# jayleicn/ClipBERT

Measured on NVIDIA H100. Metric: clips/sec fwd+bwd MSRVTT ret (ResNet50+BERT-base), higher is better.
Workload: dtype bf16

## Files before the change

clipbert_b200/csrc/common.cuh:

```cuda
#pragma once
#include <cuda.h>
#include <cuda_bf16.h>
#include <cuda_runtime.h>
#include <stdint.h>

#include "drop_cfg.h"

namespace cb {

#ifndef CB_SPIN_LIMIT
#define CB_SPIN_LIMIT (1u << 24)
#endif

__device__ __forceinline__ uint32_t smem_u32(const void* p) {
  return static_cast<uint32_t>(__cvta_generic_to_shared(p));
}

__device__ __forceinline__ void pdl_wait() { asm volatile("griddepcontrol.wait;" ::: "memory"); }
__device__ __forceinline__ void pdl_trigger() { asm volatile("griddepcontrol.launch_dependents;" ::: "memory"); }

__device__ __forceinline__ void mbar_init(uint64_t* bar, uint32_t count) {
  asm volatile("mbarrier.init.shared::cta.b64 [%0], %1;" ::"r"(smem_u32(bar)), "r"(count));
}
__device__ __forceinline__ void fence_mbar_init() {
// ... 28 lines not shown
}
__device__ __forceinline__ void mbar_wait(uint64_t* bar, uint32_t parity) {
  uint32_t spins = 0;
  while (!mbar_try_wait(bar, parity)) {
    if (++spins > CB_SPIN_LIMIT) __trap();
  }
}
__device__ __forceinline__ void mbar_wait_unguarded(uint64_t* bar, uint32_t parity) {
  while (!mbar_try_wait(bar, parity)) {
  }
}

__device__ __forceinline__ void tma_prefetch_desc(const CUtensorMap* map) {
  asm volatile("prefetch.tensormap [%0];" ::"l"(map) : "memory");
}
__device__ __forceinline__ void tma_load_2d(void* smem_dst, const CUtensorMap* map, uint64_t* bar,
                                            int c0, int c1) {
  asm volatile(
      "cp.async.bulk.tensor.2d.shared::cluster.global.mbarrier::complete_tx::bytes "
      "[%0], [%1, {%3, %4}], [%2];" ::"r"(smem_u32(smem_dst)),
      "l"(map), "r"(smem_u32(bar)), "r"(c0), "r"(c1)
      : "memory");
}

__device__ __forceinline__ void bulk_load_1d(uint32_t smem_dst, const void* gsrc, uint32_t bytes, uint64_t* bar) {
  asm volatile("cp.async.bulk.shared::cluster.global.mbarrier::complete_tx::bytes [%0], [%1], %2, [%3];" ::"r"(smem_dst), "l"(gsrc),
               "r"(bytes), "r"(smem_u32(bar))
               : "memory");
}

__device__ __forceinline__ void tma_load_2d_s32(uint32_t smem_dst, const CUtensorMap* map, uint64_t* bar, int c0, int c1) {
  asm volatile(
      "cp.async.bulk.tensor.2d.shared::cluster.global.mbarrier::complete_tx::bytes "
      "[%0], [%1, {%3, %4}], [%2];" ::"r"(smem_dst),
      "l"(map), "r"(smem_u32(bar)), "r"(c0), "r"(c1)
      : "memory");
}

__device__ __forceinline__ void tma_load_3d(void* smem_dst, const CUtensorMap* map, uint64_t* bar, int c0, int c1, int c2) {
  asm volatile(
      "cp.async.bulk.tensor.3d.shared::cluster.global.mbarrier::complete_tx::bytes "
      "[%0], [%1, {%3, %4, %5}], [%2];" ::"r"(smem_u32(smem_dst)),
      "l"(map), "r"(smem_u32(bar)), "r"(c0), "r"(c1), "r"(c2)
      : "memory");
}

__device__ __forceinline__ void tma_store_2d(const CUtensorMap* map, const void* smem_src, int c0, int c1) {
  asm volatile("cp.async.bulk.tensor.2d.global.shared::cta.bulk_group [%0, {%2, %3}], [%1];" ::"l"(map),
               "r"(smem_u32(smem_src)), "r"(c0), "r"(c1)
               : "memory");
}
__device__ __forceinline__ void tma_store_2d_s32(const CUtensorMap* map, uint32_t smem_src, int c0, int c1) {
  asm volatile("cp.async.bulk.tensor.2d.global.shared::cta.bulk_group [%0, {%2, %3}], [%1];" ::"l"(map), "r"(smem_src), "r"(c0), "r"(c1)
               : "memory");
}
__device__ __forceinline__ uint4 lds128(uint32_t saddr) {
  uint4 v;
  asm volatile("ld.shared.v4.u32 {%0, %1, %2, %3}, [%4];" : "=r"(v.x), "=r"(v.y), "=r"(v.z), "=r"(v.w) : "r"(saddr));
  return v;
}
__device__ __forceinline__ void sts128(uint32_t saddr, uint4 v) {
  asm volatile("st.shared.v4.u32 [%0], {%1, %2, %3, %4};" ::"r"(saddr), "r"(v.x), "r"(v.y), "r"(v.z), "r"(v.w) : "memory");
}
__device__ __forceinline__ void tma_store_commit() { asm volatile("cp.async.bulk.commit_group;" ::: "memory"); }
template <int N>
__device__ __forceinline__ void tma_store_wait_read() {
  asm volatile("cp.async.bulk.wait_group.read %0;" ::"n"(N) : "memory");
}
template <int N>
__device__ __forceinline__ void tma_store_wait_all() {
  asm volatile("cp.async.bulk.wait_group %0;" ::"n"(N) : "memory");
}
__device__ __forceinline__ void named_bar_sync(uint32_t id, uint32_t nthreads) {
  asm volatile("bar.sync %0, %1;" ::"r"(id), "r"(nthreads) : "memory");
}
__device__ __forceinline__ void named_bar_arrive(uint32_t id, uint32_t nthreads) {
  asm volatile("bar.arrive %0, %1;" ::"r"(id), "r"(nthreads) : "memory");
}
template <uint32_t NREG>
__device__ __forceinline__ void setmaxnreg_dec() {
  asm volatile("setmaxnreg.dec.sync.aligned.u32 %0;" ::"n"(NREG));
}
template <uint32_t NREG>
__device__ __forceinline__ void setmaxnreg_inc() {
  asm volatile("setmaxnreg.inc.sync.aligned.u32 %0;" ::"n"(NREG));
}

__device__ __forceinline__ void wgmma_fence() { asm volatile("wgmma.fence.sync.aligned;" ::: "memory"); }
__device__ __forceinline__ void wgmma_commit() { asm volatile("wgmma.commit_group.sync.aligned;" ::: "memory"); }
template <int N>
__device__ __forceinline__ void wgmma_wait() {
  asm volatile("wgmma.wait_group.sync.aligned %0;" ::"n"(N) : "memory");
}
template <int R>
__device__ __forceinline__ void wgmma_fence_acc(float (&d)[R]) {
#pragma unroll
  for (int i = 0; i < R; ++i) asm volatile("" : "+f"(d[i])::"memory");
}

__device__ __forceinline__ uint64_t gmma_desc(uint32_t smem_addr, uint32_t lbo, uint32_t sbo) {
  uint64_t d = 0;
  d |= static_cast<uint64_t>((smem_addr & 0x3FFFFu) >> 4);
  d |= static_cast<uint64_t>((lbo >> 4) & 0x3FFFu) << 16;
  d |= static_cast<uint64_t>((sbo >> 4) & 0x3FFFu) << 32;
  d |= 1ull << 62;
  return d;
// ... 183 lines not shown
```

clipbert_b200/csrc/gemm.cu:

```cuda
#include <algorithm>

#include "common.cuh"
#include "host_util.h"

namespace cb {

constexpr int BM = 128;
constexpr int BK = 64;
constexpr int CONSUMER_WARPS = 8;
constexpr int GEMM_THREADS = (CONSUMER_WARPS + 1) * 32;
constexpr int PP_THREADS = 3 * 128;
constexpr int PP_PRODUCER_REGS = 40;
constexpr int PP_CONSUMER_REGS = 232;
constexpr int PP_BAR_TURN = 1;
constexpr int MAX_STAGES = 8;
constexpr int SMEM_LIMIT = 232448;
constexpr int STG_PITCH = 36;
constexpr int STG_WARP_FLOATS = 16 * STG_PITCH;
constexpr int EPI_BYTES = CONSUMER_WARPS * STG_WARP_FLOATS * 4;
constexpr int IN_BOX_BYTES = BM * 64 * 2;

struct GemmEpi {
  const float* scale;
  const float* shift;
  const __nv_bfloat16* residual;
  const __nv_bfloat16* aux;
  int aux_mode;
  int act;
  void* out;
  int64_t out_ld;
  int out_fp32;
  __nv_bfloat16* out2;
  int64_t out2_ld;
  int rowmap, H, W;
  uint32_t drop_thresh;
  float drop_inv_keep;
  uint64_t seed;
  const uint64_t* seed_off;
  int mn3d;
  long long* dbg;
};

__device__ __forceinline__ void dbg_stamp(const GemmEpi& epi, int slot) {
  if (epi.dbg) {
    epi.dbg[blockIdx.x * 32 + slot] = clock64();
    if (slot == 0 || slot == 11) {
      unsigned long long ns;
      asm volatile("mov.u64 %0, %%globaltimer;" : "=l"(ns));
      epi.dbg[blockIdx.x * 32 + (slot == 0 ? 12 : 13)] = static_cast<long long>(ns);
    }
  }
}

template <int BN>
struct GemmCfg {
  static constexpr int A_BYTES = BM * BK * 2;
  static constexpr int B_BYTES = BN * BK * 2;
  static constexpr int STAGE_BYTES = A_BYTES + B_BYTES;
  static constexpr int BAR_BYTES = 256;
};

enum { EK_GENERIC = 0, EK_SHIFT_ACT = 1, EK_RELU_MASK = 2, EK_DROP_RES = 3, EK_GELU_STASH = 4, EK_AUX_MUL = 5 };

template <int NC>
__device__ __forceinline__ void add_shift(float (&f)[NC], const float (&shv)[NC]) {
#pragma unroll
  for (int j = 0; j < NC; ++j) f[j] += shv[j];
}
template <int NC>
__device__ __forceinline__ void add_residual(float (&f)[NC], const uint32_t (&res16)[NC / 2]) {
#pragma unroll
  for (int j = 0; j < NC / 2; ++j) {
    const float2 r2 = unpack_bf16x2(res16[j]);
    f[2 * j] += r2.x;
    f[2 * j + 1] += r2.y;
  }
}
template <int NC>
__device__ __forceinline__ void epilogue_shift_act(float (&f)[NC], const float (&shv)[NC], bool has_shift, const uint32_t (&res16)[NC / 2], bool has_res,
                                                   bool relu) {
  if (has_shift) add_shift<NC>(f, shv);
  if (has_res) add_residual<NC>(f, res16);
  if (relu) {
#pragma unroll
    for (int j = 0; j < NC; ++j) f[j] = fmaxf(f[j], 0.0f);
  }
}
template <int NC>
__device__ __forceinline__ void epilogue_relu_mask(float (&f)[NC], const uint32_t (&res16)[NC / 2], bool has_res, const uint32_t (&aux16)[NC / 2]) {
  if (has_res) add_residual<NC>(f, res16);
#pragma unroll
  for (int j = 0; j < NC / 2; ++j) {
    const uint32_t a = aux16[j];
    f[2 * j] = ((a & 0x8000u) == 0u && (a & 0x7fffu) != 0u) ? f[2 * j] : 0.0f;
    f[2 * j + 1] = ((a & 0x80000000u) == 0u && (a & 0x7fff0000u) != 0u) ? f[2 * j + 1] : 0.0f;
  }
}
template <int NC>
__device__ __forceinline__ void epilogue_drop_res(float (&f)[NC], const float (&shv)[NC], bool has_shift, const uint32_t (&res16)[NC / 2], bool has_res,
                                                  uint64_t dseed, uint64_t didx, uint32_t thresh, float inv_keep) {
  if (has_shift) add_shift<NC>(f, shv);
#pragma unroll
  for (int j = 0; j < NC; j += 4) {
    float m[4];
    dropout_mult4(dseed, didx + j, thresh, inv_keep, m);
// ... 200 lines not shown
    for (int ch = 0; ch < nch; ++ch) {
      const uint32_t a_addr = smem0 + s * stage_bytes + ch * Cfg::STAGE_BYTES;
      const uint32_t b_addr = a_addr + Cfg::A_BYTES;
#pragma unroll
      for (int k = 0; k < BK / 16; ++k) {
        const uint64_t bd = TB ? gmma_desc(b_addr + k * 2048, BK * 128, 1024) : gmma_desc(b_addr + k * 32, 16, 1024);
        const uint32_t accum = (i > 0 || ch > 0 || k > 0) ? 1u : 0u;
#pragma unroll
        for (int h = 0; h < 2; ++h) wgmma_bf16<BN, 0, TB>(acc[h], gmma_desc(a_addr + h * (64 * 128) + k * 32, 16, 1024), bd, accum);
      }
    }
    wgmma_commit();
    wgmma_wait<1>();
    wgmma_fence_acc(acc[0]);
    wgmma_fence_acc(acc[1]);
    if (prev >= 0) {
      __syncwarp();
      mbar_arrive_if(&empty_bar[prev], lane == 0);
    }
    prev = s;
    if (++s == STAGES) { s = 0; ph ^= 1; }
    if (pass_bar && i + KCH >= n_iters) {
      if (in_stage) mbar_wait_unguarded(&full_bar[s], ph);
      named_bar_arrive(pass_bar, 2 * 128);
    }
  }
  wgmma_wait<0>();
  wgmma_fence_acc(acc[0]);
  wgmma_fence_acc(acc[1]);
  if (prev >= 0) {
    __syncwarp();
    mbar_arrive_if(&empty_bar[prev], lane == 0);
  }
}

template <int BN, bool STORE = false>
__device__ __forceinline__ void wgrad_epilogue(const float (&acc)[BN / 2], float* obase, int64_t out_ld, const float* scale, int M, int N, int r0,
                                               int n0, int lane) {
  const int r1 = r0 + 8;
  const float rs0 = (r0 < M && scale) ? scale[r0] : 1.0f;
  const float rs1 = (r1 < M && scale) ? scale[r1] : 1.0f;
#pragma unroll
  for (int j = 0; j < BN / 8; ++j) {
    const int n = n0 + j * 8 + 2 * (lane & 3);
    if (n < N) {
      if constexpr (STORE) {
        if (r0 < M) *reinterpret_cast<float2*>(obase + static_cast<int64_t>(r0) * out_ld + n) = make_float2(acc[4 * j] * rs0, acc[4 * j + 1] * rs0);
        if (r1 < M) *reinterpret_cast<float2*>(obase + static_cast<int64_t>(r1) * out_ld + n) = make_float2(acc[4 * j + 2] * rs1, acc[4 * j + 3] * rs1);
      } else {
        if (r0 < M) red_add_f32x2(obase + static_cast<int64_t>(r0) * out_ld + n, acc[4 * j] * rs0, acc[4 * j + 1] * rs0);
        if (r1 < M) red_add_f32x2(obase + static_cast<int64_t>(r1) * out_ld + n, acc[4 * j + 2] * rs1, acc[4 * j + 3] * rs1);
      }
    }
  }
}

__device__ __forceinline__ uint32_t swz128(uint32_t box, int r, int q) { return box + r * 128 + ((q ^ (r & 7)) << 4); }

template <int BN, int MODE>
__global__ void __launch_bounds__(PP_THREADS, 1)
    gemm_pingpong_kernel(const __grid_constant__ CUtensorMap tmA, const __grid_constant__ CUtensorMap tmB, const __grid_constant__ CUtensorMap tmR,
                         const __grid_constant__ CUtensorMap tmX, int M, int N, int K, int ntaps, int tap_w, int tap_sign, int tiles_m,
                         int tiles_n, int total_tiles, int STAGES, int KCH, int N_IN, GemmEpi epi) {
  static_assert(MODE != 1 && BN <= 128, "TN / NN tiles of 128 x 64 or 128 x 128");
  using Cfg = GemmCfg<BN>;
  extern __shared__ uint8_t smem_raw[];
  uint8_t* smem = reinterpret_cast<uint8_t*>((reinterpret_cast<uintptr_t>(smem_raw) + 1023) & ~static_cast<uintptr_t>(1023));
  const int stage_bytes = KCH * Cfg::STAGE_BYTES;
  const bool has_res = epi.residual != nullptr, has_aux = epi.aux != nullptr;
  constexpr int IN_TILE_BYTES = (BN / 64) * IN_BOX_BYTES;
  const int in_bytes = (has_res + has_aux) * IN_TILE_BYTES;
  uint8_t* in_base = smem + STAGES * stage_bytes;
  uint8_t* stg_base = in_base + N_IN * in_bytes;
  uint64_t* full_bar = reinterpret_cast<uint64_t*>(stg_base + EPI_BYTES);
  uint64_t* empty_bar = full_bar + MAX_STAGES;
  uint64_t* in_full = empty_bar + MAX_STAGES;
  uint64_t* in_empty = in_full + 2;

  const int warp = __shfl_sync(0xffffffffu, static_cast<int>(threadIdx.x >> 5), 0);
  const int lane = threadIdx.x & 31;
  const int unit = blockIdx.x;
  const int n_units = gridDim.x;
  if (threadIdx.x == 0) dbg_stamp(epi, 0);
  pdl_trigger();
  if (threadIdx.x == 0) {
    tma_prefetch_desc(&tmA);
    tma_prefetch_desc(&tmB);
    if (has_res) tma_prefetch_desc(&tmR);
    if (has_aux) tma_prefetch_desc(&tmX);
    for (int s = 0; s < STAGES; ++s) {
      mbar_init(&full_bar[s], 1);
      mbar_init(&empty_bar[s], 4);
    }
    for (int b = 0; b < 2; ++b) {
      mbar_init(&in_full[b], 1);
      mbar_init(&in_empty[b], 4);
    }
    fence_mbar_init();
  }
  __syncthreads();
  const int kc_per_tap = (K + BK - 1) / BK;
  const int n_iters = ntaps * kc_per_tap;
  const bool in_stage = in_bytes && !N_IN;
  const int tile_stages = (n_iters + KCH - 1) / KCH + (in_stage ? 1 : 0);
  pdl_wait();
  if (threadIdx.x == 0) dbg_stamp(epi, 1);
// ... 189 lines not shown
            float4 s4 = make_float4(0.f, 0.f, 0.f, 0.f);
            if (nb + j + 4 <= N) s4 = __ldg(reinterpret_cast<const float4*>(epi.shift + nb + j));
            shv[j] = s4.x; shv[j + 1] = s4.y; shv[j + 2] = s4.z; shv[j + 3] = s4.w;
          }
        }
        uint32_t o2_16[NC / 2];
        switch (kind) {
          case EK_SHIFT_ACT: epilogue_shift_act<NC>(f, shv, has_shift, res16, has_res, kind_relu); break;
          case EK_RELU_MASK: epilogue_relu_mask<NC>(f, res16, has_res, aux16); break;
          case EK_DROP_RES:
            epilogue_drop_res<NC>(f, shv, has_shift, res16, has_res, dseed, static_cast<uint64_t>(orow) * static_cast<uint64_t>(N) + nb,
                                  epi.drop_thresh, epi.drop_inv_keep);
            break;
          case EK_GELU_STASH: epilogue_gelu_stash<NC>(f, shv, has_shift, o2_16); break;
          case EK_AUX_MUL: epilogue_aux_mul<NC>(f, res16, has_res, aux16); break;
          default:
            if (guard) epilogue_math<NC, true>(f, epi, shv, has_shift, dseed, nb, N, orow, res16, has_res, aux16, has_aux, o2_16, has_out2);
            else epilogue_math<NC, false>(f, epi, shv, has_shift, dseed, nb, N, orow, res16, has_res, aux16, has_aux, o2_16, has_out2);
        }
        if (epi.out_fp32) {
          float* o = reinterpret_cast<float*>(epi.out) + orow * epi.out_ld + nb;
#pragma unroll
          for (int j = 0; j < NC; j += 4)
            if (nb + j + 4 <= N) *reinterpret_cast<float4*>(o + j) = make_float4(f[j], f[j + 1], f[j + 2], f[j + 3]);
        } else {
          __nv_bfloat16* o = reinterpret_cast<__nv_bfloat16*>(epi.out) + orow * epi.out_ld + nb;
#pragma unroll
          for (int j = 0; j < 2; ++j)
            if (nb + 8 * j + 8 <= N)
              *reinterpret_cast<uint4*>(o + 8 * j) = make_uint4(pack_bf16x2(f[8 * j], f[8 * j + 1]), pack_bf16x2(f[8 * j + 2], f[8 * j + 3]),
                                                                pack_bf16x2(f[8 * j + 4], f[8 * j + 5]), pack_bf16x2(f[8 * j + 6], f[8 * j + 7]));
        }
        if (has_out2) {
          __nv_bfloat16* o = epi.out2 + orow * epi.out2_ld + nb;
#pragma unroll
          for (int j = 0; j < 2; ++j)
            if (nb + 8 * j + 8 <= N) *reinterpret_cast<uint4*>(o + 8 * j) = make_uint4(o2_16[4 * j], o2_16[4 * j + 1], o2_16[4 * j + 2], o2_16[4 * j + 3]);
        }
      }
    }
    if (in_bytes) {
      __syncwarp();
      if (lane == 0) mbar_arrive(N_IN ? &in_empty[N_IN == 2 ? wg : 0] : &empty_bar[s]);
      if (!N_IN && ++s == STAGES) { s = 0; ph ^= 1; }
    }
    ring_skip(tile_stages);
  }
  if (threadIdx.x == 4 * 32) dbg_stamp(epi, 11);
}

template <int BN, bool DET = false>
__global__ void __launch_bounds__(GEMM_THREADS, 1)
    gemm_kernel(const __grid_constant__ CUtensorMap tmA, const __grid_constant__ CUtensorMap tmB, int M, int N, int K, int ntaps, int tap_w,
                int tap_sign, int iters_per_split, int tiles_m, int tiles_n, int total_tiles, int STAGES, int KCH, GemmEpi epi, float* ws) {
  using Cfg = GemmCfg<BN>;
  extern __shared__ uint8_t smem_raw[];
  uint8_t* smem = reinterpret_cast<uint8_t*>((reinterpret_cast<uintptr_t>(smem_raw) + 1023) & ~static_cast<uintptr_t>(1023));
  const int stage_bytes = KCH * Cfg::STAGE_BYTES;
  uint64_t* full_bar = reinterpret_cast<uint64_t*>(smem + STAGES * stage_bytes);
  uint64_t* empty_bar = full_bar + MAX_STAGES;

  const int warp = __shfl_sync(0xffffffffu, static_cast<int>(threadIdx.x >> 5), 0);
  const int lane = threadIdx.x & 31;
  const int unit = blockIdx.x;
  const int n_units = gridDim.x;
  if (threadIdx.x == 0) dbg_stamp(epi, 0);
  pdl_trigger();
  if (threadIdx.x == 0) {
    tma_prefetch_desc(&tmA);
    tma_prefetch_desc(&tmB);
    for (int s = 0; s < STAGES; ++s) {
      mbar_init(&full_bar[s], 1);
      mbar_init(&empty_bar[s], CONSUMER_WARPS);
    }
    fence_mbar_init();
  }
  __syncthreads();
  pdl_wait();
  if (threadIdx.x == 0) dbg_stamp(epi, 1);

  if (warp >= CONSUMER_WARPS) {
    if (warp == CONSUMER_WARPS && lane == 0) {
      int s = 0;
      uint32_t ph = 0;
      for (int tile = unit; tile < total_tiles; tile += n_units) {
        const TileInfo t = decode_tile<BN, 1>(tile, tiles_m, tiles_n, K, ntaps, iters_per_split);
        int shift = 0;
        if (ntaps == 9) shift = tap_sign * ((t.tap / 3 - 1) * tap_w + (t.tap % 3 - 1));
        for (int i = 0; i < t.n_iters; i += KCH) {
          const int nch = min(KCH, t.n_iters - i);
          mbar_wait(&empty_bar[s], ph ^ 1);
          mbar_expect_tx(&full_bar[s], nch * Cfg::STAGE_BYTES);
          int kit = t.it_begin + i;
          for (int ch = 0; ch < nch; ++ch, ++kit) {
            uint8_t* sa = smem + s * stage_bytes + ch * Cfg::STAGE_BYTES;
            uint8_t* sb = sa + Cfg::A_BYTES;
            const int p = kit * BK;
            if (epi.mn3d) {
              tma_load_3d(sa, &tmA, &full_bar[s], 0, p, t.m0 >> 6);
              tma_load_3d(sb, &tmB, &full_bar[s], 0, p + shift, t.nb0 >> 6);
            } else {
#pragma unroll
              for (int j = 0; j < BM / 64; ++j) tma_load_2d(sa + j * (BK * 128), &tmA, &full_bar[s], t.m0 + j * 64, p);
#pragma unroll
              for (int j = 0; j < BN / 64; ++j) tma_load_2d(sb + j * (BK * 128), &tmB, &full_bar[s], t.nb0 + j * 64, p + shift);
            }
          }
          if (++s == STAGES) { s = 0; ph ^= 1; }
          if (i == 0 && tile == unit) dbg_stamp(epi, 2);
        }
      }
      dbg_stamp(epi, 3);
    }
    return;
  }

  const int wg = warp >> 2;
  const int wrow = wg * 64 + (warp & 3) * 16;
  const uint32_t smem0 = smem_u32(smem);
  float acc[BN / 2];
  int s = 0;
  uint32_t ph = 0;
  int local = 0;
  for (int tile = unit; tile < total_tiles; tile += n_units, ++local) {
    const TileInfo t = decode_tile<BN, 1>(tile, tiles_m, tiles_n, K, ntaps, iters_per_split);
    if (local == 0 && warp == 0 && lane == 0) dbg_stamp(epi, 4);
    mma_tile<BN, 1, 1>(acc, smem0, stage_bytes, KCH, STAGES, t.n_iters, wg, lane, s, ph, full_bar, empty_bar);
    if (local == 0 && warp == 0 && lane == 0) dbg_stamp(epi, 5);
    if constexpr (DET)
      wgrad_epilogue<BN, true>(acc, ws + static_cast<int64_t>(t.it_begin / iters_per_split) * M * ntaps * N + static_cast<int64_t>(t.tap) * N,
                               static_cast<int64_t>(ntaps) * N, epi.scale, M, N, t.m0 + wrow + (lane >> 2), t.n0, lane);
    else
      wgrad_epilogue<BN>(acc, reinterpret_cast<float*>(epi.out) + static_cast<int64_t>(t.tap) * N, epi.out_ld, epi.scale, M, N,
                         t.m0 + wrow + (lane >> 2), t.n0, lane);
    if (local == 0 && warp == 0 && lane == 0) dbg_stamp(epi, 8);
  }
  if (threadIdx.x == 0) dbg_stamp(epi, 11);
}

static int g_sm_limit = 0;
static int sm_count_device() {
  static int n = 0;
  if (n == 0) {
    int dev = 0;
    cudaGetDevice(&dev);
    cudaDeviceGetAttribute(&n, cudaDevAttrMultiProcessorCount, dev);
    if (n <= 0) n = 132;
  }
  return n;
}
static int sm_count() {
  const int n = sm_count_device();
  return (g_sm_limit > 0 && g_sm_limit < n) ? g_sm_limit : n;
}
static int plan_sm_count() { return g_det.load(std::memory_order_relaxed) ? sm_count_device() : sm_count(); }

static long long* g_gemm_timeline = nullptr;
static int g_force_kch = 0;
static int g_mn3d = 1;


struct SmemPlan {
  int epi_bytes, kch, stages, chunk_bytes, n_in;
};
static SmemPlan plan_ring(int bn, bool staging, int kiters, int force_kch, int in_bytes, int n_in) {
  SmemPlan p;
  const int limit = SMEM_LIMIT;
  p.chunk_bytes = BM * BK * 2 + bn * BK * 2;
  p.epi_bytes = staging ? EPI_BYTES : 0;
  p.n_in = n_in;
  const int chunks_fit = (limit - 1024 - GemmCfg<64>::BAR_BYTES - p.epi_bytes - n_in * in_bytes) / p.chunk_bytes;
  const int min_stages = kiters > chunks_fit ? 3 : 2;
  p.kch = 1;
  if (force_kch > 0) p.kch = force_kch;
  else if (g_force_kch > 0) p.kch = g_force_kch;
  else if (kiters >= 4 && chunks_fit >= 4 * min_stages) p.kch = 4;
  else if (kiters >= 2 && chunks_fit >= 2 * min_stages) p.kch = 2;
  if (p.kch > kiters) p.kch = kiters;
  if (p.kch > 1 && chunks_fit / p.kch < 2) p.kch = 1;
  p.stages = chunks_fit / p.kch;
  if (p.stages > MAX_STAGES) p.stages = MAX_STAGES;
  const int stage_iters = ceil_div(kiters, p.kch);
  const int cap = staging ? 2 * stage_iters + 1 : (stage_iters + 1 > 2 ? stage_iters + 1 : 2);
  if (p.stages > cap) p.stages = cap;
  return p;
}
static SmemPlan plan_smem(int bn, bool staging, int kiters, int force_kch = 0, int in_bytes = 0) {
  const SmemPlan none = plan_ring(bn, staging, kiters, force_kch, 0, 0);
  if (in_bytes == 0) return none;
  const SmemPlan two = plan_ring(bn, staging, kiters, force_kch, in_bytes, 2);
  if (two.stages >= 2 && two.stages * two.kch >= kiters) return two;
  if (kiters > 4 && none.stages >= 2 && none.kch * none.chunk_bytes >= in_bytes) return none;
  return plan_ring(bn, staging, kiters, force_kch, in_bytes, 1);
}
static int epi_in_bytes(const cb_gemm_desc& d, int bn) {
  return d.mode == CB_GEMM_WGRAD ? 0 : ((d.residual != nullptr) + (d.aux != nullptr)) * (bn / 64) * IN_BOX_BYTES;
}

static int real_splits(int kc, int want) {
  const int sp = want < 1 ? 1 : (want > kc ? kc : want);
  return ceil_div(kc, ceil_div(kc, sp));
}

struct SplitReduceJob {
  float* out;
  const float* ws;
  int64_t out_ld;
  int M, W, S;
};
struct SplitReduce {
  int njobs;
  SplitReduceJob j[8];
};
__global__ void __launch_bounds__(256) wgrad_split_reduce_kernel(const __grid_constant__ SplitReduce r) {
  pdl_wait();
  pdl_trigger();
  const SplitReduceJob& J = r.j[blockIdx.y];
  const int w4 = J.W / 4;
  const int64_t total = static_cast<int64_t>(J.M) * w4, plane = static_cast<int64_t>(J.M) * J.W;
  for (int64_t i = static_cast<int64_t>(blockIdx.x) * 256 + threadIdx.x; i < total; i += static_cast<int64_t>(gridDim.x) * 256) {
    const int64_t m = i / w4;
    const int c = static_cast<int>(i - m * w4) * 4;
    float4* o = reinterpret_cast<float4*>(J.out + m * J.out_ld + c);
    float4 v = *o;
    const float* p = J.ws + m * J.W + c;
    for (int s = 0; s < J.S; ++s) {
      const float4 a = *reinterpret_cast<const float4*>(p + s * plane);
      v.x += a.x; v.y += a.y; v.z += a.z; v.w += a.w;
    }
    *o = v;
  }
}
static int launch_split_reduce(const SplitReduce& r, cudaStream_t stream, const char* what) {
  int64_t most = 0;
  for (int i = 0; i < r.njobs; ++i) most = std::max(most, static_cast<int64_t>(r.j[i].M) * (r.j[i].W / 4));
  const int gx = static_cast<int>(std::min<int64_t>(1024, (most + 255) / 256));
  launch_k(wgrad_split_reduce_kernel, dim3(gx, r.njobs), 256, 0, stream, r);
  return check_launch(what);
}

template <int BN, int MODE, bool DET = false>
static int launch_gemm(const cb_gemm_desc& d, const GemmEpi& epi_in, cudaStream_t stream, float* ws = nullptr) {
  static_assert(MODE == 1 || BN <= 128, "TN / NN: 128 x 64 or 128 x 128 tiles");
  static_assert(MODE == 1 || !DET, "only the weight gradients have a deterministic instantiation");
  GemmEpi epi = epi_in;
  using Cfg = GemmCfg<BN>;
  static bool attr_set = false;
  auto kern = [] {
    if constexpr (MODE == 1) return gemm_kernel<BN, DET>;
    else return gemm_pingpong_kernel<BN, MODE>;
  }();
  if (!attr_set) {
    cudaError_t e = cudaFuncSetAttribute(kern, cudaFuncAttributeMaxDynamicSharedMemorySize, SMEM_LIMIT);
    if (e != cudaSuccess) {
      set_error("cudaFuncSetAttribute(smem=%d): %s", SMEM_LIMIT, cudaGetErrorString(e));
      return CB_ERR_CUDA;
    }
    attr_set = true;
  }
  alignas(64) CUtensorMap ta, tb, tr, tx;
  bool mn3d = false;
  int iters_per_split = 0;
  const int tiles_m = ceil_div(d.m, BM), tiles_n = ceil_div(d.n, BN);
  int total = tiles_m * tiles_n;
  int kiters;
  bool ok;
  if (MODE == 0) {
    ok = get_tmap_2d(&ta, d.a, d.k, d.a_rows, d.a_ld, BK, BM) &&
         get_tmap_2d(&tb, d.b, static_cast<uint64_t>(d.k) * d.ntaps, d.b_rows, d.b_ld, BK, BN);
    kiters = ceil_div(d.k, BK) * d.ntaps;
  } else if (MODE == 2) {
    ok = get_tmap_2d(&ta, d.a, d.k, d.a_rows, d.a_ld, BK, BM);
    mn3d = g_mn3d && d.n % 64 == 0 &&
           get_tmap_3d_mn(&tb, d.b, static_cast<uint64_t>(d.n) * d.ntaps, d.b_rows, d.b_ld, BK, BN / 64);
    if (!mn3d) ok = ok && get_tmap_2d(&tb, d.b, static_cast<uint64_t>(d.n) * d.ntaps, d.b_rows, d.b_ld, 64, BK);
    kiters = ceil_div(d.k, BK) * d.ntaps;
  } else {
    mn3d = g_mn3d && d.m % 64 == 0 && d.n % 64 == 0 && get_tmap_3d_mn(&ta, d.a, d.m, d.a_rows, d.a_ld, BK, BM / 64) &&
           get_tmap_3d_mn(&tb, d.b, d.n, d.b_rows, d.b_ld, BK, BN / 64);
    ok = mn3d || (get_tmap_2d(&ta, d.a, d.m, d.a_rows, d.a_ld, 64, BK) && get_tmap_2d(&tb, d.b, d.n, d.b_rows, d.b_ld, 64, BK));
    const int kc = ceil_div(d.k, BK);
    iters_per_split = ceil_div(kc, real_splits(kc, d.split_k));
    total *= real_splits(kc, d.split_k) * d.ntaps;
    kiters = iters_per_split;
  }
  tr = ta;
  tx = ta;
  if (MODE != 1 && d.residual) ok = ok && get_tmap_2d(&tr, d.residual, d.n, d.m, d.res_ld, 64, BM);
  if (MODE != 1 && d.aux) ok = ok && get_tmap_2d(&tx, d.aux, d.n, d.m, d.aux_ld, 64, BM);
  if (!ok) return CB_ERR_CUDA;
  epi.mn3d = mn3d ? 1 : 0;
  const int units = sm_count();
  const int grid = total < units ? total : units;
  const int in_bytes = epi_in_bytes(d, BN);
  const SmemPlan sp = plan_smem(BN, MODE != 1, kiters, (d.reserved >> 8) & 15, in_bytes);
  const int kch = sp.kch, stages = sp.stages;
  if (stages < 2) {
    set_error("cb_gemm: not enough shared memory for a 2-stage pipeline (BN=%d, epilogue %d B + inputs %d B)", BN, sp.epi_bytes,
              in_bytes);
    return CB_ERR_INVALID;
  }
  const int smem_bytes = stages * kch * Cfg::STAGE_BYTES + sp.n_in * in_bytes + sp.epi_bytes + Cfg::BAR_BYTES + 1024;
  if constexpr (MODE == 1)
    launch_gemm_k(kern, grid, GEMM_THREADS, smem_bytes, stream, ta, tb, d.m, d.n, d.k, d.ntaps, d.tap_w, d.tap_sign, iters_per_split,
                  tiles_m, tiles_n, total, stages, kch, epi, ws);
  else
    launch_gemm_k(kern, grid, PP_THREADS, smem_bytes, stream, ta, tb, tr, tx, d.m, d.n, d.k, d.ntaps, d.tap_w, d.tap_sign, tiles_m,
                  tiles_n, total, stages, kch, sp.n_in, epi);
  return check_launch("cb_gemm");
}

struct LaunchCfg {
  int bn, splits;
};

static LaunchCfg choose_config(const cb_gemm_desc& d, int units) {
  const int kc = ceil_div(d.k, BK);
  const bool wgrad = d.mode == CB_GEMM_WGRAD;
  const int block_n = (!wgrad && d.block_n == 256) ? 128 : d.block_n;
  static const int cand[3] = {64, 128, 256};
  LaunchCfg best = {64, 1};
  double best_cost = 1e30;
  for (int c = 0; c < 3; ++c) {
    const int bn = cand[c];
    if (block_n && bn != block_n) continue;
    if (!wgrad && bn == 256) continue;
    if (bn > 64 && d.n <= bn / 2) continue;
    const int64_t base = static_cast<int64_t>(ceil_div(d.m, BM)) * ceil_div(d.n, bn) * (wgrad ? d.ntaps : 1);
    const int max_split = wgrad ? (d.split_k > 0 ? d.split_k : (kc < 32 ? kc : 32)) : 1;
    for (int sp = (wgrad && d.split_k > 0) ? d.split_k : 1; sp <= max_split; ++sp) {
      const int ips = ceil_div(wgrad ? kc : kc * d.ntaps, sp);
      const int real_sp = wgrad ? ceil_div(kc, ips) : 1;
      const int64_t tiles = base * real_sp;
      const double rounds = static_cast<double>((tiles + units - 1) / units);
      const SmemPlan pl = plan_smem(bn, !wgrad, ips, (d.reserved >> 8) & 15, epi_in_bytes(d, bn));
      if (pl.stages < 2) continue;
      const double shallow = (pl.stages * pl.kch < 3 && ips > 2) ? 3.0 : 1.0;
      const double stage_cost = 450.0 + pl.kch * pl.chunk_bytes / 60.0;
      const double main_loop = ceil_div(ips, pl.kch) * stage_cost * shallow;
      double cost;
      if (wgrad) {
        cost = rounds * (main_loop + bn * 24.0) + 2500.0;
      } else {
        const double epi = bn * 30.0;
        const double per_tile = main_loop > 0.5 * (main_loop + epi) ? main_loop : 0.5 * (main_loop + epi);
        cost = rounds * per_tile + 0.5 * epi + 2500.0;
      }
      if (cost < best_cost) {
        best_cost = cost;
        best = {bn, real_sp};
      }
    }
  }
  return best;
}

constexpr int WG_MAX_PROBLEMS = 8;
struct WgradProblem {
  CUtensorMap tmA, tmB;
  float* out;
  const float* scale;
  int64_t out_ld;
  int M, N, K;
  int ntaps, tap_w, tap_sign;
  int iters_per_split, tiles_m, tiles_n;
  int tile_begin;
  int mn3d;
};
struct WgradGroup {
  int nprob, total_tiles;
  WgradProblem p[WG_MAX_PROBLEMS];
};
struct WgradWorkspace {
  float* p[WG_MAX_PROBLEMS];
};
struct WgTile {
  int pi, m0, n0, tap, it_begin, n_iters;
};
__device__ __forceinline__ WgTile wg_decode(const WgradGroup& g, int tile) {
  WgTile t;
  int pi = 0;
  while (pi + 1 < g.nprob && tile >= g.p[pi + 1].tile_begin) ++pi;
  const WgradProblem& P = g.p[pi];
  int r = tile - P.tile_begin;
  const int nt = r % P.tiles_n;
  r /= P.tiles_n;
  const int mt = r % P.tiles_m;
  r /= P.tiles_m;
  t.pi = pi;
  t.m0 = mt * BM;
  t.tap = r % P.ntaps;
  const int split = r / P.ntaps;
  const int kc = (P.K + BK - 1) / BK;
  t.it_begin = split * P.iters_per_split;
  t.n_iters = min(kc, t.it_begin + P.iters_per_split) - t.it_begin;
  t.n0 = nt;
  return t;
}

template <int BN, bool DET = false>
__global__ void __launch_bounds__(GEMM_THREADS, 1)
    wgrad_group_kernel(const __grid_constant__ WgradGroup g, int STAGES, int KCH, const __grid_constant__ WgradWorkspace ws) {
  using Cfg = GemmCfg<BN>;
  extern __shared__ uint8_t smem_raw[];
  uint8_t* smem = reinterpret_cast<uint8_t*>((reinterpret_cast<uintptr_t>(smem_raw) + 1023) & ~static_cast<uintptr_t>(1023));
  const int stage_bytes = KCH * Cfg::STAGE_BYTES;
  uint64_t* full_bar = reinterpret_cast<uint64_t*>(smem + STAGES * stage_bytes);
  uint64_t* empty_bar = full_bar + MAX_STAGES;
  const int warp = __shfl_sync(0xffffffffu, static_cast<int>(threadIdx.x >> 5), 0);
  const int lane = threadIdx.x & 31;
  const int unit = blockIdx.x, n_units = gridDim.x;
  pdl_trigger();
  if (threadIdx.x == 0) {
    for (int i = 0; i < g.nprob; ++i) {
      tma_prefetch_desc(&g.p[i].tmA);
      tma_prefetch_desc(&g.p[i].tmB);
    }
    for (int s = 0; s < STAGES; ++s) {
      mbar_init(&full_bar[s], 1);
      mbar_init(&empty_bar[s], CONSUMER_WARPS);
    }
    fence_mbar_init();
  }
  __syncthreads();
  pdl_wait();

  if (warp >= CONSUMER_WARPS) {
    if (warp == CONSUMER_WARPS && lane == 0) {
      int s = 0;
      uint32_t ph = 0;
      for (int tile = unit; tile < g.total_tiles; tile += n_units) {
        const WgTile t = wg_decode(g, tile);
        const WgradProblem& P = g.p[t.pi];
        const int n0 = t.n0 * BN;
        int shift = 0;
        if (P.ntaps == 9) shift = P.tap_sign * ((t.tap / 3 - 1) * P.tap_w + (t.tap % 3 - 1));
        for (int i = 0; i < t.n_iters; i += KCH) {
          const int nch = min(KCH, t.n_iters - i);
          mbar_wait(&empty_bar[s], ph ^ 1);
          mbar_expect_tx(&full_bar[s], nch * Cfg::STAGE_BYTES);
          int kit = t.it_begin + i;
          for (int ch = 0; ch < nch; ++ch, ++kit) {
            uint8_t* sa = smem + s * stage_bytes + ch * Cfg::STAGE_BYTES;
            uint8_t* sb = sa + Cfg::A_BYTES;
            const int p = kit * BK;
            if (P.mn3d) {
              tma_load_3d(sa, &P.tmA, &full_bar[s], 0, p, t.m0 >> 6);
              tma_load_3d(sb, &P.tmB, &full_bar[s], 0, p + shift, n0 >> 6);
            } else {
#pragma unroll
              for (int j = 0; j < BM / 64; ++j) tma_load_2d(sa + j * (BK * 128), &P.tmA, &full_bar[s], t.m0 + j * 64, p);
#pragma unroll
              for (int j = 0; j < BN / 64; ++j) tma_load_2d(sb + j * (BK * 128), &P.tmB, &full_bar[s], n0 + j * 64, p + shift);
            }
          }
          if (++s == STAGES) { s = 0; ph ^= 1; }
        }
      }
    }
    return;
  }

  const int wg = warp >> 2;
  const int wrow = wg * 64 + (warp & 3) * 16;
  const uint32_t smem0 = smem_u32(smem);
  float acc[BN / 2];
  int s = 0;
  uint32_t ph = 0;
  for (int tile = unit; tile < g.total_tiles; tile += n_units) {
    const WgTile t = wg_decode(g, tile);
    const WgradProblem& P = g.p[t.pi];
    mma_tile<BN, 1, 1>(acc, smem0, stage_bytes, KCH, STAGES, t.n_iters, wg, lane, s, ph, full_bar, empty_bar);
    if (DET && ws.p[t.pi] != nullptr)
      wgrad_epilogue<BN, true>(acc, ws.p[t.pi] + static_cast<int64_t>(t.it_begin / P.iters_per_split) * P.M * P.ntaps * P.N +
                                        static_cast<int64_t>(t.tap) * P.N,
                               static_cast<int64_t>(P.ntaps) * P.N, P.scale, P.M, P.N, t.m0 + wrow + (lane >> 2), t.n0 * BN, lane);
    else
      wgrad_epilogue<BN>(acc, P.out + static_cast<int64_t>(t.tap) * P.N, P.out_ld, P.scale, P.M, P.N, t.m0 + wrow + (lane >> 2), t.n0 * BN, lane);
  }
}

template <int BN, bool DET = false>
static int launch_wgrad_group(const cb_gemm_desc* descs, int n, int splits, cudaStream_t stream, float* ws = nullptr) {
  using Cfg = GemmCfg<BN>;
  static bool attr_set = false;
  auto kern = wgrad_group_kernel<BN, DET>;
  if (!attr_set) {
    cudaError_t e = cudaFuncSetAttribute(kern, cudaFuncAttributeMaxDynamicSharedMemorySize, SMEM_LIMIT);
    if (e != cudaSuccess) {
      set_error("cudaFuncSetAttribute(smem=%d): %s", SMEM_LIMIT, cudaGetErrorString(e));
      return CB_ERR_CUDA;
    }
    attr_set = true;
  }
  alignas(64) WgradGroup g;
  g.nprob = n;
  SplitReduce red;
  red.njobs = 0;
  WgradWorkspace wsp;
  int total = 0, max_iters = 0;
  for (int i = 0; i < n; ++i) {
    const cb_gemm_desc& d = descs[i];
    WgradProblem& P = g.p[i];
    const bool mn3d = g_mn3d && d.m % 64 == 0 && d.n % 64 == 0 && get_tmap_3d_mn(&P.tmA, d.a, d.m, d.a_rows, d.a_ld, BK, BM / 64) &&
                      get_tmap_3d_mn(&P.tmB, d.b, d.n, d.b_rows, d.b_ld, BK, BN / 64);
    if (!mn3d && !(get_tmap_2d(&P.tmA, d.a, d.m, d.a_rows, d.a_ld, 64, BK) && get_tmap_2d(&P.tmB, d.b, d.n, d.b_rows, d.b_ld, 64, BK)))
      return CB_ERR_CUDA;
    P.mn3d = mn3d ? 1 : 0;
    P.out = static_cast<float*>(d.out);
    P.scale = d.scale;
    P.out_ld = d.out_ld;
    P.M = d.m; P.N = d.n; P.K = d.k;
    P.ntaps = d.ntaps; P.tap_w = d.tap_w; P.tap_sign = d.tap_sign;
    const int kc = ceil_div(d.k, BK);
    const int sp = real_splits(kc, splits);
    P.iters_per_split = ceil_div(kc, sp);
    wsp.p[i] = nullptr;
    if (DET && sp > 1) {
      wsp.p[i] = ws;
      red.j[red.njobs++] = {static_cast<float*>(d.out), ws, d.out_ld, d.m, d.ntaps * d.n, sp};
      ws += static_cast<int64_t>(sp) * d.m * d.ntaps * d.n;
    }
    P.tiles_m = ceil_div(d.m, BM);
    P.tiles_n = ceil_div(d.n, BN);
    P.tile_begin = total;
    total += P.tiles_m * P.tiles_n * d.ntaps * sp;
    if (P.iters_per_split > max_iters) max_iters = P.iters_per_split;
  }
  g.total_tiles = total;
  const SmemPlan sp = plan_smem(BN, false, max_iters);
  if (sp.stages < 2) {
    set_error("cb_gemm_wgrad_group: not enough shared memory for a 2-stage pipeline (BN=%d)", BN);
    return CB_ERR_INVALID;
  }
  const int smem_bytes = sp.stages * sp.kch * Cfg::STAGE_BYTES + Cfg::BAR_BYTES + 1024;
  const int units = sm_count();
  launch_gemm_k(kern, total < units ? total : units, GEMM_THREADS, smem_bytes, stream, g, sp.stages, sp.kch, wsp);
  const int rc = check_launch("cb_gemm_wgrad_group");
  if (rc != CB_OK || red.njobs == 0) return rc;
  return launch_split_reduce(red, stream, "cb_gemm_wgrad_group(split reduce)");
}

struct GroupPlan {
  bool groupable;
  int bn, split;
};
static GroupPlan group_plan(const cb_gemm_desc* descs, int n, int sms) {
  GroupPlan gp = {n >= 2 && n <= WG_MAX_PROBLEMS, 64, 1};
  for (int i = 0; i < n; ++i)
    if (descs[i].k * 2 < descs[0].k || descs[0].k * 2 < descs[i].k) gp.groupable = false;
  if (!gp.groupable) return gp;
  int min_n = descs[0].n;
  for (int i = 1; i < n; ++i) min_n = descs[i].n < min_n ? descs[i].n : min_n;
  gp.bn = descs[0].block_n ? descs[0].block_n : (min_n >= 192 ? 256 : (min_n >= 96 ? 128 : 64));
  int64_t base = 0;
  int kc_min = 1 << 30, kc_max = 0;
  for (int i = 0; i < n; ++i) {
    base += static_cast<int64_t>(ceil_div(descs[i].m, BM)) * ceil_div(descs[i].n, gp.bn) * descs[i].ntaps;
    const int kc = ceil_div(descs[i].k, BK);
    kc_min = kc < kc_min ? kc : kc_min;
    kc_max = kc > kc_max ? kc : kc_max;
  }
  double best_cost = 1e30;
  for (int sp = 1; sp <= 8 && sp <= kc_min; ++sp) {
    const double waves = static_cast<double>((base * sp + sms - 1) / sms);
    const double cost = waves * (ceil_div(kc_max, sp) + 8.0);
    if (cost < best_cost) { best_cost = cost; gp.split = sp; }
  }
  if (descs[0].split_k > 0) gp.split = descs[0].split_k;
  return gp;
}

static int64_t wgrad_ws_bytes(const cb_gemm_desc& d, int splits) {
  return splits > 1 ? static_cast<int64_t>(splits) * d.m * d.ntaps * d.n * 4 : 0;
}
static int64_t group_ws_bytes(const cb_gemm_desc* descs, int n) {
  const GroupPlan gp = group_plan(descs, n, sm_count_device());
  int64_t bytes = 0;
  for (int i = 0; i < n; ++i) {
    const int64_t b = gp.groupable ? wgrad_ws_bytes(descs[i], real_splits(ceil_div(descs[i].k, BK), gp.split))
                                   : wgrad_ws_bytes(descs[i], choose_config(descs[i], sm_count_device()).splits);
    bytes = gp.groupable ? bytes + b : std::max(bytes, b);
  }
  return bytes;
}

}

extern "C" void cb_debug_gemm_timeline(void* device_buf) { cb::g_gemm_timeline = static_cast<long long*>(device_buf); }
extern "C" void cb_debug_gemm_kch(int kch) { cb::g_force_kch = kch; }
// ... 158 lines not shown
```

Before: 3973.

## Use bulk async reduce-add from shared staging for wgrad split-K epilogue

Replaces per-thread red.global.add f32x2 atomics in the wgrad epilogue with a per-warp shared-memory staging slab (double-buffered, rotated to avoid bank conflicts) followed by cp.reduce.async.bulk add.f32 per row. The aim is to cut the number of global atomic transactions and let the reduction overlap with the next tile's MMA. It takes shared memory from the pipeline ring for staging, which may reduce the number of stages, and it adds debug timeline stamps to the group kernel.

```diff
diff --git a/clipbert_b200/csrc/common.cuh b/clipbert_b200/csrc/common.cuh
--- a/clipbert_b200/csrc/common.cuh
+++ b/clipbert_b200/csrc/common.cuh
@@ -104,6 +104,10 @@
 }
 __device__ __forceinline__ void tma_store_2d_s32(const CUtensorMap* map, uint32_t smem_src, int c0, int c1) {
   asm volatile("cp.async.bulk.tensor.2d.global.shared::cta.bulk_group [%0, {%2, %3}], [%1];" ::"l"(map), "r"(smem_src), "r"(c0), "r"(c1)
+               : "memory");
+}
+__device__ __forceinline__ void bulk_reduce_add_f32(float* gdst, uint32_t smem_src, uint32_t bytes) {
+  asm volatile("cp.reduce.async.bulk.global.shared::cta.bulk_group.add.f32 [%0], [%1], %2;" ::"l"(gdst), "r"(smem_src), "r"(bytes)
                : "memory");
 }
 __device__ __forceinline__ uint4 lds128(uint32_t saddr) {
diff --git a/clipbert_b200/csrc/gemm.cu b/clipbert_b200/csrc/gemm.cu
--- a/clipbert_b200/csrc/gemm.cu
+++ b/clipbert_b200/csrc/gemm.cu
@@ -51,6 +51,16 @@
     }
   }
 }
+__device__ __forceinline__ void dbg_stamp(long long* dbg, int slot) {
+  if (dbg) {
+    dbg[blockIdx.x * 32 + slot] = clock64();
+    if (slot == 0 || slot == 11) {
+      unsigned long long ns;
+      asm volatile("mov.u64 %0, %%globaltimer;" : "=l"(ns));
+      dbg[blockIdx.x * 32 + (slot == 0 ? 12 : 13)] = static_cast<long long>(ns);
+    }
+  }
+}
 
 template <int BN>
 struct GemmCfg {
@@ -357,6 +367,55 @@
         if (r1 < M) red_add_f32x2(obase + static_cast<int64_t>(r1) * out_ld + n, acc[4 * j + 2] * rs1, acc[4 * j + 3] * rs1);
       }
     }
+  }
+}
+
+constexpr int WG_SLAB_COLS = 32;
+constexpr int WG_SLAB_BYTES = 16 * WG_SLAB_COLS * 4;
+constexpr int WG_STAGING_BYTES = CONSUMER_WARPS * 2 * WG_SLAB_BYTES;
+
+__device__ __forceinline__ void sts64(uint32_t saddr, float x, float y) {
+  asm volatile("st.shared.v2.f32 [%0], {%1, %2};" ::"r"(saddr), "f"(x), "f"(y) : "memory");
+}
+
+template <int BN>
+__device__ __forceinline__ void wgrad_epilogue_bulk(const float (&acc)[BN / 2], float* obase, int64_t out_ld, const float* scale, int M, int N,
+                                                    int row0, int n0, int lane, uint32_t slabs) {
+  const int r = lane >> 2, rot = r & 3;
+  const int r0 = row0 + r, r1 = r0 + 8;
+  const float rs0 = (r0 < M && scale) ? scale[r0] : 1.0f;
+  const float rs1 = (r1 < M && scale) ? scale[r1] : 1.0f;
+  const bool issuer = lane < 16 && row0 + lane < M;
+  float* grow = obase + static_cast<int64_t>(row0 + lane) * out_ld + n0;
+  const uint32_t st0 = slabs + r * (WG_SLAB_COLS * 4) + (lane & 3) * 8;
+#pragma unroll
+  for (int sl = 0; sl < BN / WG_SLAB_COLS; ++sl) {
+    const uint32_t buf = (sl & 1) * WG_SLAB_BYTES;
+    if (lane < 16) tma_store_wait_read<1>();
+    __syncwarp();
+    float a[4][4], b[4][4];
+#pragma unroll
+    for (int t = 0; t < 4; ++t) {
+      const int j = sl * 4 + t;
+      a[t][0] = acc[4 * j] * rs0; a[t][1] = acc[4 * j + 1] * rs0;
+      a[t][2] = acc[4 * j + 2] * rs1; a[t][3] = acc[4 * j + 3] * rs1;
+    }
+#pragma unroll
+    for (int t = 0; t < 4; ++t)
+#pragma unroll
+      for (int e = 0; e < 4; ++e) b[t][e] = (rot & 1) ? a[(t + 1) & 3][e] : a[t][e];
+#pragma unroll
+    for (int t = 0; t < 4; ++t) {
+      const uint32_t dst = st0 + buf + ((t + rot) & 3) * 32;
+      sts64(dst, (rot & 2) ? b[(t + 2) & 3][0] : b[t][0], (rot & 2) ? b[(t + 2) & 3][1] : b[t][1]);
+      sts64(dst + 8 * (WG_SLAB_COLS * 4), (rot & 2) ? b[(t + 2) & 3][2] : b[t][2], (rot & 2) ? b[(t + 2) & 3][3] : b[t][3]);
+    }
+    fence_proxy_async_smem();
+    __syncwarp();
+    const int n = n0 + sl * WG_SLAB_COLS;
+    if (issuer && n < N)
+      bulk_reduce_add_f32(grow + sl * WG_SLAB_COLS, slabs + buf + lane * (WG_SLAB_COLS * 4), min(WG_SLAB_COLS, N - n) * 4);
+    if (lane < 16) tma_store_commit();
   }
 }
 
@@ -652,7 +711,7 @@
 template <int BN, bool DET = false>
 __global__ void __launch_bounds__(GEMM_THREADS, 1)
     gemm_kernel(const __grid_constant__ CUtensorMap tmA, const __grid_constant__ CUtensorMap tmB, int M, int N, int K, int ntaps, int tap_w,
-                int tap_sign, int iters_per_split, int tiles_m, int tiles_n, int total_tiles, int STAGES, int KCH, GemmEpi epi, float* ws) {
+                int tap_sign, int iters_per_split, int tiles_m, int tiles_n, int total_tiles, int STAGES, int KCH, GemmEpi epi, float* ws, int bulk_epi) {
   using Cfg = GemmCfg<BN>;
   extern __shared__ uint8_t smem_raw[];
   uint8_t* smem = reinterpret_cast<uint8_t*>((reinterpret_cast<uintptr_t>(smem_raw) + 1023) & ~static_cast<uintptr_t>(1023));
@@ -718,6 +777,7 @@
   const int wg = warp >> 2;
   const int wrow = wg * 64 + (warp & 3) * 16;
   const uint32_t smem0 = smem_u32(smem);
+  const uint32_t slabs = smem0 + STAGES * stage_bytes + Cfg::BAR_BYTES + warp * (2 * WG_SLAB_BYTES);
   float acc[BN / 2];
   int s = 0;
   uint32_t ph = 0;
@@ -730,12 +790,19 @@
     if constexpr (DET)
       wgrad_epilogue<BN, true>(acc, ws + static_cast<int64_t>(t.it_begin / iters_per_split) * M * ntaps * N + static_cast<int64_t>(t.tap) * N,
                                static_cast<int64_t>(ntaps) * N, epi.scale, M, N, t.m0 + wrow + (lane >> 2), t.n0, lane);
+    else if (bulk_epi)
+      wgrad_epilogue_bulk<BN>(acc, reinterpret_cast<float*>(epi.out) + static_cast<int64_t>(t.tap) * N, epi.out_ld, epi.scale, M, N,
+                              t.m0 + wrow, t.n0, lane, slabs);
     else
       wgrad_epilogue<BN>(acc, reinterpret_cast<float*>(epi.out) + static_cast<int64_t>(t.tap) * N, epi.out_ld, epi.scale, M, N,
                          t.m0 + wrow + (lane >> 2), t.n0, lane);
     if (local == 0 && warp == 0 && lane == 0) dbg_stamp(epi, 8);
   }
-  if (threadIdx.x == 0) dbg_stamp(epi, 11);
+  if (!DET && bulk_epi && lane < 16) tma_store_wait_all<0>();
+  if (threadIdx.x == 0) {
+    dbg_stamp(epi, 11);
+    if (epi.dbg) epi.dbg[blockIdx.x * 32 + 14] = local;
+  }
 }
 
 static int g_sm_limit = 0;
@@ -793,6 +860,11 @@
   if (kiters > 4 && none.stages >= 2 && none.kch * none.chunk_bytes >= in_bytes) return none;
   return plan_ring(bn, staging, kiters, force_kch, in_bytes, 1);
 }
+static SmemPlan plan_wgrad(int bn, int kiters, int force_kch, bool bulk) {
+  return plan_ring(bn, false, kiters, force_kch, bulk ? WG_STAGING_BYTES : 0, 1);
+}
+constexpr int RESERVED_RED_EPILOGUE = 1 << 12;
+static bool wgrad_bulk(const cb_gemm_desc& d) { return !g_det.load(std::memory_order_relaxed) && !(d.reserved & RESERVED_RED_EPILOGUE); }
 static int epi_in_bytes(const cb_gemm_desc& d, int bn) {
   return d.mode == CB_GEMM_WGRAD ? 0 : ((d.residual != nullptr) + (d.aux != nullptr)) * (bn / 64) * IN_BOX_BYTES;
 }
@@ -892,8 +964,9 @@
   epi.mn3d = mn3d ? 1 : 0;
   const int units = sm_count();
   const int grid = total < units ? total : units;
-  const int in_bytes = epi_in_bytes(d, BN);
-  const SmemPlan sp = plan_smem(BN, MODE != 1, kiters, (d.reserved >> 8) & 15, in_bytes);
+  const bool bulk = MODE == 1 && !DET && wgrad_bulk(d);
+  const int in_bytes = MODE == 1 ? (bulk ? WG_STAGING_BYTES : 0) : epi_in_bytes(d, BN);
+  const SmemPlan sp = MODE == 1 ? plan_wgrad(BN, kiters, (d.reserved >> 8) & 15, bulk) : plan_smem(BN, true, kiters, (d.reserved >> 8) & 15, in_bytes);
   const int kch = sp.kch, stages = sp.stages;
   if (stages < 2) {
     set_error("cb_gemm: not enough shared memory for a 2-stage pipeline (BN=%d, epilogue %d B + inputs %d B)", BN, sp.epi_bytes,
@@ -903,7 +976,7 @@
   const int smem_bytes = stages * kch * Cfg::STAGE_BYTES + sp.n_in * in_bytes + sp.epi_bytes + Cfg::BAR_BYTES + 1024;
   if constexpr (MODE == 1)
     launch_gemm_k(kern, grid, GEMM_THREADS, smem_bytes, stream, ta, tb, d.m, d.n, d.k, d.ntaps, d.tap_w, d.tap_sign, iters_per_split,
-                  tiles_m, tiles_n, total, stages, kch, epi, ws);
+                  tiles_m, tiles_n, total, stages, kch, epi, ws, bulk ? 1 : 0);
   else
     launch_gemm_k(kern, grid, PP_THREADS, smem_bytes, stream, ta, tb, tr, tx, d.m, d.n, d.k, d.ntaps, d.tap_w, d.tap_sign, tiles_m,
                   tiles_n, total, stages, kch, sp.n_in, epi);
@@ -933,7 +1006,8 @@
       const int real_sp = wgrad ? ceil_div(kc, ips) : 1;
       const int64_t tiles = base * real_sp;
       const double rounds = static_cast<double>((tiles + units - 1) / units);
-      const SmemPlan pl = plan_smem(bn, !wgrad, ips, (d.reserved >> 8) & 15, epi_in_bytes(d, bn));
+      const SmemPlan pl = wgrad ? plan_wgrad(bn, ips, (d.reserved >> 8) & 15, wgrad_bulk(d))
+                                : plan_smem(bn, true, ips, (d.reserved >> 8) & 15, epi_in_bytes(d, bn));
       if (pl.stages < 2) continue;
       const double shallow = (pl.stages * pl.kch < 3 && ips > 2) ? 3.0 : 1.0;
       const double stage_cost = 450.0 + pl.kch * pl.chunk_bytes / 60.0;
@@ -1000,7 +1074,8 @@
 
 template <int BN, bool DET = false>
 __global__ void __launch_bounds__(GEMM_THREADS, 1)
-    wgrad_group_kernel(const __grid_constant__ WgradGroup g, int STAGES, int KCH, const __grid_constant__ WgradWorkspace ws) {
+    wgrad_group_kernel(const __grid_constant__ WgradGroup g, int STAGES, int KCH, const __grid_constant__ WgradWorkspace ws, int bulk_epi,
+                       long long* dbg) {
   using Cfg = GemmCfg<BN>;
   extern __shared__ uint8_t smem_raw[];
   uint8_t* smem = reinterpret_cast<uint8_t*>((reinterpret_cast<uintptr_t>(smem_raw) + 1023) & ~static_cast<uintptr_t>(1023));
@@ -1010,6 +1085,7 @@
   const int warp = __shfl_sync(0xffffffffu, static_cast<int>(threadIdx.x >> 5), 0);
   const int lane = threadIdx.x & 31;
   const int unit = blockIdx.x, n_units = gridDim.x;
+  if (threadIdx.x == 0) dbg_stamp(dbg, 0);
   pdl_trigger();
   if (threadIdx.x == 0) {
     for (int i = 0; i < g.nprob; ++i) {
@@ -1064,19 +1140,31 @@
   const int wg = warp >> 2;
   const int wrow = wg * 64 + (warp & 3) * 16;
   const uint32_t smem0 = smem_u32(smem);
+  const uint32_t slabs = smem0 + STAGES * stage_bytes + Cfg::BAR_BYTES + warp * (2 * WG_SLAB_BYTES);
   float acc[BN / 2];
   int s = 0;
   uint32_t ph = 0;
-  for (int tile = unit; tile < g.total_tiles; tile += n_units) {
+  int local = 0;
+  for (int tile = unit; tile < g.total_tiles; tile += n_units, ++local) {
     const WgTile t = wg_decode(g, tile);
     const WgradProblem& P = g.p[t.pi];
+    if (local == 0 && warp == 0 && lane == 0) dbg_stamp(dbg, 4);
     mma_tile<BN, 1, 1>(acc, smem0, stage_bytes, KCH, STAGES, t.n_iters, wg, lane, s, ph, full_bar, empty_bar);
+    if (local == 0 && warp == 0 && lane == 0) dbg_stamp(dbg, 5);
     if (DET && ws.p[t.pi] != nullptr)
       wgrad_epilogue<BN, true>(acc, ws.p[t.pi] + static_cast<int64_t>(t.it_begin / P.iters_per_split) * P.M * P.ntaps * P.N +
                                         static_cast<int64_t>(t.tap) * P.N,
                                static_cast<int64_t>(P.ntaps) * P.N, P.scale, P.M, P.N, t.m0 + wrow + (lane >> 2), t.n0 * BN, lane);
+    else if (!DET && bulk_epi)
+      wgrad_epilogue_bulk<BN>(acc, P.out + static_cast<int64_t>(t.tap) * P.N, P.out_ld, P.scale, P.M, P.N, t.m0 + wrow, t.n0 * BN, lane, slabs);
     else
       wgrad_epilogue<BN>(acc, P.out + static_cast<int64_t>(t.tap) * P.N, P.out_ld, P.scale, P.M, P.N, t.m0 + wrow + (lane >> 2), t.n0 * BN, lane);
+    if (local == 0 && warp == 0 && lane == 0) dbg_stamp(dbg, 8);
+  }
+  if (!DET && bulk_epi && lane < 16) tma_store_wait_all<0>();
+  if (threadIdx.x == 0) {
+    dbg_stamp(dbg, 11);
+    if (dbg) dbg[blockIdx.x * 32 + 14] = local;
   }
 }
 
@@ -1128,14 +1216,16 @@
     if (P.iters_per_split > max_iters) max_iters = P.iters_per_split;
   }
   g.total_tiles = total;
-  const SmemPlan sp = plan_smem(BN, false, max_iters);
+  const bool bulk = !DET && wgrad_bulk(descs[0]);
+  const SmemPlan sp = plan_wgrad(BN, max_iters, 0, bulk);
   if (sp.stages < 2) {
     set_error("cb_gemm_wgrad_group: not enough shared memory for a 2-stage pipeline (BN=%d)", BN);
     return CB_ERR_INVALID;
   }
-  const int smem_bytes = sp.stages * sp.kch * Cfg::STAGE_BYTES + Cfg::BAR_BYTES + 1024;
+  const int smem_bytes = sp.stages * sp.kch * Cfg::STAGE_BYTES + (bulk ? WG_STAGING_BYTES : 0) + Cfg::BAR_BYTES + 1024;
   const int units = sm_count();
-  launch_gemm_k(kern, total < units ? total : units, GEMM_THREADS, smem_bytes, stream, g, sp.stages, sp.kch, wsp);
+  launch_gemm_k(kern, total < units ? total : units, GEMM_THREADS, smem_bytes, stream, g, sp.stages, sp.kch, wsp, bulk ? 1 : 0,
+                g_gemm_timeline);
   const int rc = check_launch("cb_gemm_wgrad_group");
   if (rc != CB_OK || red.njobs == 0) return rc;
   return launch_split_reduce(red, stream, "cb_gemm_wgrad_group(split reduce)");
```

Result: no change. 3997 (median of 6 runs) (+0.6%).
